# theouterlimitz/Audio-Mastering-Engine

Hardware: AMD Instinct MI355X
Metric: mastered Msamples/sec (48 kHz stereo f32) at 1/2/4/8 GPUs; % HBM roofline (higher is better)
Workload: dtype f64

## Files before the change

### audio-mastering-engine_amd/csrc/amx_dyn.hip

```cpp
#include "amx_dev.hpp"

namespace amx {

typedef double d2v __attribute__((ext_vector_type(2)));
typedef uint32_t u4v __attribute__((ext_vector_type(4)));

#define AMX_TAB 32769

#define AMX_RMS_N 4096
#define AMX_RMS_MAXLOOK 1024

__device__ __forceinline__ int rms_slot(int k) { return k + (k >> 4); }

__device__ __forceinline__ uint32_t rms_floor(uint64_t S, uint32_t cnt, double rc) {
    const double sd = fma((double)(uint32_t)(S >> 32), 4294967296.0, (double)(uint32_t)S);
    const double cd = (double)cnt;
    const uint32_t k = (uint32_t)__builtin_amdgcn_sqrtf((float)(sd * rc));
    const uint32_t k1 = k + 1;
    const bool up = (double)__umul24(k1, k1) * cd <= sd;
    const bool down = (double)__umul24(k, k) * cd > sd;
    const uint32_t r = k + (uint32_t)up - (uint32_t)(down & !up);
    return cnt ? (r > 32768u ? 32768u : r) : 0u;
}

// ... 267 lines not shown
__device__ __forceinline__ void env0_tile(const ChainDev &cd, double *sm, double (&G)[16],
                                          u2v (&Islot)[4], const u2v (&Inext)[4],
                                          const uint16_t *const (&irow)[4], const double *mt, int q,
                                          int ntile, int nwarm, int64_t start, int64_t end,
                                          double *ckr, double &att, double &s_spec, bool &any) {
    const int lane = threadIdx.x & 63;
#pragma unroll
    for (int i = 0; i < 4; i++) {
        double *d = sm + ((lane >> 2) + 16 * i) * AMX_ENV_MP + 4 * (lane & 3);
        *reinterpret_cast<d2v *>(d) = d2v{G[4 * i], G[4 * i + 1]};
        *reinterpret_cast<d2v *>(d + 2) = d2v{G[4 * i + 2], G[4 * i + 3]};
    }
    __builtin_amdgcn_wave_barrier();
    {
        const int qn = (q + AMX_ENV_PF < ntile ? q + AMX_ENV_PF : q) * AMX_ENV_TF;
#pragma unroll
        for (int i = 0; i < 4; i++) Islot[i] = *reinterpret_cast<const u2v *>(irow[i] + qn);
        env_gather(mt, Inext, G);
    }
    const int64_t f0 = start + (int64_t)q * AMX_ENV_TF;
    const bool in = f0 >= 0 && f0 < end;
    double mv[AMX_ENV_TF];
#pragma unroll
    for (int i = 0; i < 8; i++) {
        const d2v v = *reinterpret_cast<const d2v *>(sm + lane * AMX_ENV_MP + 2 * i);
        mv[2 * i] = v.x;
        mv[2 * i + 1] = v.y;
    }
    __builtin_amdgcn_wave_barrier();
    if (q == nwarm) s_spec = att;
    if (in) {
        if (q >= nwarm) {
            ckr[f0 / AMX_ENV_TF] = att;
            uint32_t h = 0, l = 0;
#pragma unroll
            for (int f = 0; f < AMX_ENV_TF; f++) {
                const unsigned long long x = (unsigned long long)__double_as_longlong(mv[f]);
                h |= (uint32_t)(x >> 32);
                l |= (uint32_t)x;
            }
            any |= ((h & 0x7fffffffu) | l) != 0u;
        }
        double iv[AMX_ENV_TF], dv[AMX_ENV_TF];
#pragma unroll
        for (int f = 0; f < AMX_ENV_TF; f++) {
            iv[f] = env_div<RCP>(mv[f], cd.env_A, cd.env_rA);
            dv[f] = env_div<RCP>(mv[f], cd.env_R, cd.env_rR);
        }
#pragma unroll
        for (int f = 0; f < AMX_ENV_TF; f++) att = env_step3(att, mv[f], iv[f], dv[f]);
    }
}

#define AMX_ENV_WG 4
#define AMX_ENV_LDS_PIN (48 * 1024)
template <bool RCP>
__global__ void __launch_bounds__(64 * AMX_ENV_WG) k_env0(const ChainDev *__restrict__ cdp,
                                             const ChunkDev *__restrict__ chunks,
                                             const SegDev *__restrict__ es, int n_es,
                                             const uint16_t *__restrict__ mi,
                                             const double *__restrict__ tabs,
                                             double *__restrict__ ck,
                                             double *__restrict__ sv, double *__restrict__ ev,
                                             int *__restrict__ act, int64_t nloc, int warm,
                                             int *__restrict__ flags) {
    __shared__ __attribute__((aligned(16))) double sm_all[AMX_ENV_WG][64 * AMX_ENV_MP];
    const ChainDev &cd = *cdp;
    const int lane = threadIdx.x & 63, wv = __builtin_amdgcn_readfirstlane(threadIdx.x >> 6);
    double *sm = sm_all[wv];
    if (blockIdx.x == 0 && blockIdx.y == 0 && threadIdx.x < AMX_ENV_MAX_ROUNDS) flags[threadIdx.x] = 0;
    if (blockIdx.x == 0 && blockIdx.y == 0 && threadIdx.x < 64) {
        for (int k = lane; k < AMX_ENV_MAX_ROUNDS * AMX_ENV_NCTR; k += 64) flags[AMX_ENV_MAX_ROUNDS + k] = 0;
        if (lane < 3) flags[AMX_ENV_LIST + lane] = 0;
    }
    const EnvBands eb = env_bands(flags + AMX_ENV_BACT);
    if ((int)blockIdx.y >= eb.nb) return;
    const int b = env_slot_band(eb, blockIdx.y);
    es += cd.etab[eb.nb].es_off;
    n_es = cd.etab[eb.nb].n_es;
    const int Le = cd.etab[eb.nb].Le, ld = cd.es_ld;
    if ((int)(blockIdx.x * (blockDim.x >> 6)) * 64 >= n_es) return;
    const int j = (blockIdx.x * (blockDim.x >> 6) + wv) * 64 + lane;
    const bool valid = j < n_es;
    const SegDev sg = es[valid ? j : n_es - 1];
    const ChunkDev ch = chunks[sg.chunk];
    const int64_t rowoff = b * nloc + ch.loc_off;
    const int64_t start = sg.pos - warm;
    const int64_t end = valid ? sg.pos + sg.len : sg.pos;
    double *ckr = ck + rowoff / AMX_ENV_TF;
    const double *mt = tabs + (int64_t)b * 3 * AMX_TAB;
    const int ntile = (warm + Le) / AMX_ENV_TF, nwarm = warm / AMX_ENV_TF;
    const uint16_t *irow[4];
#pragma unroll
    for (int i = 0; i < 4; i++) {
        const int r = 16 * i + (lane >> 2);
        irow[i] = mi + __shfl(rowoff + start, r) + 4 * (lane & 3);
    }
    u2v I[AMX_ENV_PF][4];
#pragma unroll
    for (int u = 0; u < AMX_ENV_PF; u++)
#pragma unroll
        for (int i = 0; i < 4; i++) I[u][i] = *reinterpret_cast<const u2v *>(irow[i] + u * AMX_ENV_TF);
    double G[2][16];
    env_gather(mt, I[0], G[0]);
    env_gather(mt, I[1], G[1]);
    double att = 0.0, s_spec = 0.0;
    if (cd.env_guess && start >= 0) att = mt[mi[rowoff + start]];
    bool any = false;
    for (int q0 = 0; q0 < ntile; q0 += AMX_ENV_PF) {
#pragma unroll
        for (int u = 0; u < AMX_ENV_PF; u++)
            env0_tile<RCP>(cd, sm, G[u & 1], I[u], I[(u + 2) % AMX_ENV_PF], irow, mt,
                           q0 + u, ntile, nwarm, start, end, ckr, att, s_spec, any);
    }
    if (valid) {
        sv[(int64_t)b * ld + j] = s_spec;
        ev[(int64_t)b * ld + j] = att;
        act[(int64_t)b * ld + j] = any ? 1 : 0;
    }
}

template <bool RCP>
__device__ __forceinline__ double env_fix_segment(const ChainDev &cd, const uint16_t *mrow,
                                                  const double *mt, double *ckr, int64_t pos, int len,
                                                  bool active, double ns, double old_end) {
    if (!active) {
        const int64_t k0 = pos / AMX_ENV_TF_, k1 = (pos + len + AMX_ENV_TF_ - 1) / AMX_ENV_TF_;
        for (int64_t k = k0 + (threadIdx.x & 63); k < k1; k += 64) ckr[k] = ns;
        return ns;
    }
    return env_rerun_wave<RCP>(cd, mrow, mt, ckr, pos, pos + len, ns, old_end);
}

template <bool RCP>
__global__ void __launch_bounds__(64) k_envneed(const ChainDev *__restrict__ cdp,
                                                const SegDev *__restrict__ es, int n_es,
                                                const double *__restrict__ sv,
                                                const double *__restrict__ ev,
                                                const int *__restrict__ act, int *flags,
                                                int *__restrict__ prev, int *__restrict__ list) {
    const ChainDev &cd = *cdp;
    const int b = blockIdx.y, lane = threadIdx.x;
    const EnvBands eb = env_bands(flags + AMX_ENV_BACT);
    if (!eb.act(b)) return;
    es += cd.etab[eb.nb].es_off;
    n_es = cd.etab[eb.nb].n_es;
    const int w0 = blockIdx.x * 64;
    if (w0 >= n_es) return;
    const int j = w0 + lane;
    const bool valid = j < n_es;
    const int64_t bo = (int64_t)b * cd.es_ld;
    const SegDev sg = es[valid ? j : n_es - 1];
    const bool a = valid && act[bo + j] != 0;
    const unsigned long long am = __ballot(a);
    const unsigned long long below = lane ? am & (~0ull >> (64 - lane)) : 0ull;
    int p = below ? w0 + 63 - __clzll((long long)below) : -1;
    if (p < sg.first) p = -1;
    const bool lb = valid && p < 0 && sg.first < w0;
    if (__ballot(lb)) {
        const int first0 = __shfl(sg.first, 0);
        int last = -1;
        for (int base = w0 - 64; base + 63 >= first0; base -= 64) {
            const int jj = base + lane;
            const unsigned long long mk = __ballot(jj >= first0 && act[bo + jj] != 0);
            if (mk) { last = base + 63 - __clzll((long long)mk); break; }
        }
        if (lb) p = last;
    }
    bool need = false;
    if (valid) {
        prev[bo + j] = p;
        need = !((p >= 0 ? ev[bo + p] : 0.0) == sv[bo + j]);
    }
    const unsigned long long nm = __ballot(need);
    if (nm) {
        int base = 0;
        if (lane == 0) base = atomicAdd(flags + AMX_ENV_LIST, __popcll(nm));
        base = __shfl(base, 0);
        const unsigned long long lt = lane ? ~0ull >> (64 - lane) : 0ull;
        if (need) list[base + __popcll(nm & lt)] = (int)(bo + j);
    }
}

template <bool RCP>
__global__ void __launch_bounds__(64) k_envwide(const ChainDev *__restrict__ cdp,
                                                const ChunkDev *__restrict__ chunks,
                                                const SegDev *__restrict__ es,
                                                const uint16_t *__restrict__ mm,
                                                const double *__restrict__ tabs,
                                                double *__restrict__ ck, double *sv, double *ev,
                                                const int *__restrict__ act, int *flags,
                                                const int *__restrict__ prev,
                                                const int *__restrict__ list, int64_t nloc) {
    const int count = __builtin_amdgcn_readfirstlane(flags[AMX_ENV_LIST]);
    if (blockIdx.x == 0 && threadIdx.x == 0) flags[AMX_ENV_MAX_ROUNDS + 3] = count;
    if ((int)blockIdx.x >= count) return;
    const ChainDev &cd = *cdp;
    const int lane = threadIdx.x;
    const EnvBands eb = env_bands(flags + AMX_ENV_BACT);
    const SegDev *et = es + cd.etab[eb.nb].es_off;
    const int ld = cd.es_ld;
    for (int i = blockIdx.x; i < count; i += gridDim.x) {
        const int k = __builtin_amdgcn_readfirstlane(list[i]);
        const int b = k / ld, j = k - b * ld;
        const int64_t bo = (int64_t)b * ld;
        const SegDev sg = et[j];
        const int p = prev[bo + j];
        const double ns = p >= 0 ? ev[bo + p] : 0.0;
        const int64_t ro = b * nloc + chunks[sg.chunk].loc_off;
        const double r = env_fix_segment<RCP>(cd, mm + ro, tabs + (int64_t)b * 3 * AMX_TAB, ck + ro / AMX_ENV_TF_,
                                              sg.pos, sg.len, act[bo + j] != 0, ns, ev[bo + j]);
        __builtin_amdgcn_wave_barrier();
        if (lane == 0) {
            sv[bo + j] = ns;
            ev[bo + j] = r;
        }
    }
}

#ifndef AMX_ENV_CHAIN_WAVES
#define AMX_ENV_CHAIN_WAVES 2048
#endif
template <bool RCP>
__global__ void __launch_bounds__(64) k_envheads(const ChainDev *__restrict__ cdp,
                                                 const SegDev *__restrict__ es, int n_es,
                                                 const double *__restrict__ sv,
                                                 const double *__restrict__ ev,
                                                 int *flags, int *__restrict__ list,
                                                 int *__restrict__ hmark) {
    const ChainDev &cd = *cdp;
    const int b = blockIdx.y, lane = threadIdx.x;
    const EnvBands eb = env_bands(flags + AMX_ENV_BACT);
    if (!eb.act(b)) return;
    es += cd.etab[eb.nb].es_off;
    n_es = cd.etab[eb.nb].n_es;
    if ((int)blockIdx.x * 64 >= n_es) return;
    const int j = blockIdx.x * 64 + lane;
    const int64_t bo = (int64_t)b * cd.es_ld;
    bool head = false;
    if (j < n_es) {
        const int first = es[j].first;
        const bool need = !(sv[bo + j] == (j == first ? 0.0 : ev[bo + j - 1]));
        bool needp = false;
        if (j > first) needp = !(sv[bo + j - 1] == (j - 1 == first ? 0.0 : ev[bo + j - 2]));
        head = need && !needp;
        hmark[bo + j] = head ? 1 : 0;
    }
    const unsigned long long hm = __ballot(head);
    if (hm) {
        int base = 0;
        if (lane == 0) base = atomicAdd(flags + AMX_ENV_LIST + 1, __popcll(hm));
        base = __shfl(base, 0);
        const unsigned long long below = lane ? hm & (~0ull >> (64 - lane)) : 0ull;
        if (head) list[base + __popcll(below)] = (int)(bo + j);
    }
}

template <bool RCP>
__global__ void __launch_bounds__(64) k_envchain(const ChainDev *__restrict__ cdp,
                                                 const ChunkDev *__restrict__ chunks,
                                                 const SegDev *__restrict__ es,
                                                 const uint16_t *__restrict__ mm,
                                                 const double *__restrict__ tabs,
                                                 double *__restrict__ ck, double *sv, double *ev,
                                                 const int *__restrict__ act, int *flags,
                                                 const int *__restrict__ list,
                                                 const int *__restrict__ hmark, int64_t nloc) {
    const int count = __builtin_amdgcn_readfirstlane(flags[AMX_ENV_LIST + 1]);
    if ((int)blockIdx.x >= count) return;
    const ChainDev &cd = *cdp;
    const int lane = threadIdx.x;
    const EnvBands eb = env_bands(flags + AMX_ENV_BACT);
    const SegDev *et = es + cd.etab[eb.nb].es_off;
    const int ld = cd.es_ld;
    int *ctr = flags + AMX_ENV_MAX_ROUNDS;
    int runs = 0, longest = 0, chains = 0;
    bool stale = false;
    const int n_es = cd.etab[eb.nb].n_es;
    for (int i = blockIdx.x; i < count; i += gridDim.x) {
        const int k = __builtin_amdgcn_readfirstlane(list[i]);
        const int b = k / ld, j = k - b * ld;
        const int64_t bo = (int64_t)b * ld;
        const double *mt = tabs + (int64_t)b * 3 * AMX_TAB;
        SegDev sg = et[j];
        const int64_t ro = b * nloc + chunks[sg.chunk].loc_off;
        double *ckr = ck + ro / AMX_ENV_TF_;
        double state = j == sg.first ? 0.0 : ev[bo + j - 1];
        int cur = j, walked = 0;
        bool done = false;
        while (!done) {
            const bool a = act[bo + cur] != 0;
            double old_end = ev[bo + cur];
            const double r = env_fix_segment<RCP>(cd, mm + ro, mt, ckr, sg.pos, sg.len, a, state, old_end);
            walked++;
            __builtin_amdgcn_wave_barrier();
            if (lane == 0) {
                sv[bo + cur] = state;
                ev[bo + cur] = r;
            }
            if (sg.last) break;
            int nx = cur + 1;
            while (true) {
                const int kk = nx + lane;
                const bool inch = kk < n_es && et[kk < n_es ? kk : n_es - 1].first == sg.first;
                bool hk = false, ak = false, st = true;
                double svk = 0.0, evk = 0.0;
                if (inch) {
                    hk = hmark[bo + kk] != 0;
                    ak = act[bo + kk] != 0;
                    svk = sv[bo + kk];
                    evk = ev[bo + kk];
                    st = hk || ak || svk == r;
                }
                const unsigned long long mk = __ballot(st);
                const int f = mk ? __ffsll((long long)mk) - 1 : 64;
                if (f > 0) {
                    const SegDev s0 = et[nx], s1 = et[nx + f - 1];
                    const int64_t k0 = s0.pos / AMX_ENV_TF_, k1 = (s1.pos + s1.len + AMX_ENV_TF_ - 1) / AMX_ENV_TF_;
                    for (int64_t q = k0 + lane; q < k1; q += 64) ckr[q] = r;
                    if (lane < f) {
                        sv[bo + kk] = r;
                        ev[bo + kk] = r;
                    }
                    old_end = __shfl(evk, f - 1);
                    walked += f;
                }
                if (f == 64) {
                    nx += 64;
                    continue;
                }
                const bool ins = __shfl((int)inch, f) != 0, hs = __shfl((int)hk, f) != 0;
                const double ss = __shfl(svk, f);
                if (!ins) { done = true; break; }
                if (hs) {
                    stale = stale || !(r == old_end);
                    done = true;
                    break;
                }
                if (ss == r) { done = true; break; }
                state = r;
                cur = nx + f;
                sg = et[cur];
                break;
            }
        }
        runs += walked;
        longest = walked > longest ? walked : longest;
        chains++;
    }
    if (lane == 0) {
        if (stale) flags[AMX_ENV_LIST + 2] = 1;
        atomicAdd(ctr + 0, runs);
        atomicMax(ctr + 1, longest);
        atomicAdd(ctr + 2, chains);
    }
}

template <bool RCP>
__global__ void __launch_bounds__(64) k_envseq(const ChainDev *__restrict__ cdp,
                                               const ChunkDev *__restrict__ chunks,
                                               const SegDev *__restrict__ es, int n_es,
                                               const int *__restrict__ eseg0,
                                               const int *__restrict__ neseg,
                                               const uint16_t *__restrict__ mm,
                                               const double *__restrict__ tabs,
                                               double *__restrict__ ck,
                                               double *__restrict__ sv, double *__restrict__ ev,
                                               const int *__restrict__ act, int64_t nloc,
                                               const int *__restrict__ flags, int fl) {
    if (fl >= 0 && __builtin_amdgcn_readfirstlane(flags[fl]) == 0) return;
    const ChainDev &cd = *cdp;
    const int c = blockIdx.x, b = blockIdx.y, lane = threadIdx.x;
    const EnvBands eb = env_bands(flags + AMX_ENV_BACT);
    if (!eb.act(b)) return;
    const int tb = eb.nb;
    es += cd.etab[tb].es_off;
    const int s0 = eseg0[cd.etab[tb].ch_off + c], s1 = s0 + neseg[cd.etab[tb].ch_off + c];
    const ChunkDev ch = chunks[c];
    const int64_t ld = cd.es_ld;
    double *S = sv + (int64_t)b * ld, *E = ev + (int64_t)b * ld;
    const int *A = act + (int64_t)b * ld;
    const int64_t ro = b * nloc + ch.loc_off;
    int cur = s0;
    while (cur < s1) {
        int found = s1;
        for (int base = cur; base < s1; base += 64) {
            const int j = base + lane;
            bool bad = false;
            if (j < s1) bad = !((j == s0 ? 0.0 : E[j - 1]) == S[j]);
            const unsigned long long mk = __ballot(bad);
            if (mk) { found = base + __ffsll((long long)mk) - 1; break; }
        }
        if (found >= s1) break;
        const SegDev sg = es[found];
        const double ns = found == s0 ? 0.0 : E[found - 1];
        const double r = env_fix_segment<RCP>(cd, mm + ro, tabs + (int64_t)b * 3 * AMX_TAB,
                                              ck + ro / AMX_ENV_TF_, sg.pos, sg.len, A[found] != 0,
                                              ns, E[found]);
        __syncthreads();
        if (lane == 0) {
            E[found] = r;
            S[found] = ns;
        }
        __threadfence_block();
        __syncthreads();
        cur = found + 1;
    }
}

#define AMX_GO_XP 20
#define AMX_GO_WAVES (AMX_BLOCK / 64)
template <bool RCP>
__global__ void __launch_bounds__(AMX_BLOCK) k_gain_overlay(const ChainDev *__restrict__ cdp,
                                                            const ChunkDev *__restrict__ chunks,
                                                            const uint16_t *__restrict__ mm,
                                                            const double *__restrict__ tabs,
                                                            const double *__restrict__ ck,
                                                            const uint32_t *__restrict__ bands,
                                                            uint32_t *__restrict__ out,
                                                            int64_t nloc,
                                                            const int64_t *__restrict__ n1tab,
                                                            const int *__restrict__ act,
// ... 257 lines not shown
    if (d.look > AMX_RMS_MAXLOOK || C < 1 || C > 8) return hipErrorInvalidValue;
    hipError_t e = launch_zero(bact, 3 * sizeof(int), d.st);
    if (e != hipSuccess) return e;
    const uint32_t *x = reinterpret_cast<const uint32_t *>(bands);
#define MCR(LPV)                                                                                   \
    {                                                                                              \
        constexpr int F = AMX_RMS_N - LPV;                                                         \
        dim3 g((unsigned)((d.max_chunk_n + F - 1) / F), (unsigned)d.n_chunks, 3);                  \
        if (!empty(g))                                                                             \
            hipLaunchKernelGGL(k_mc_rms<LPV>, g, dim3(AMX_BLOCK), 0, d.st, d.cd, d.chunks, schunks, x, \
                               snloc, C, m, d.nloc, bact);                                         \
    }
    if (d.look <= 256) MCR(256) else if (d.look <= 512) MCR(512) else MCR(1024)
#undef MCR
    return hipGetLastError();
}

hipError_t launch_mc_gain_overlay(const DynLaunch &d, const ChunkDev *schunks, const uint16_t *m,
                                  const double *ck, const int16_t *bands, int64_t snloc, int C,
                                  int64_t max_chunk_out, const int64_t *n1tab, const int *bact, int16_t *out) {
    dim3 g((unsigned)((max_chunk_out + AMX_ENV_TF_ * AMX_BLOCK - 1) / (AMX_ENV_TF_ * AMX_BLOCK)),
           (unsigned)d.n_chunks);
    if (empty(g)) return hipSuccess;
    const uint32_t *x = reinterpret_cast<const uint32_t *>(bands);
    if (d.rcp)
        hipLaunchKernelGGL(k_mc_gain_overlay<true>, g, dim3(AMX_BLOCK), 0, d.st, d.cd, d.chunks, schunks, m,
                           d.tabs, ck, x, snloc, d.nloc, C, n1tab, bact, out);
    else
        hipLaunchKernelGGL(k_mc_gain_overlay<false>, g, dim3(AMX_BLOCK), 0, d.st, d.cd, d.chunks, schunks, m,
                           d.tabs, ck, x, snloc, d.nloc, C, n1tab, bact, out);
    return hipGetLastError();
}

template <int LP>
static void rms_t(const DynLaunch &d, const int16_t *bands, uint16_t *m, int *bact) {
    constexpr int N = LP == 256 ? AMX_RMS_N256 : AMX_RMS_N;
    constexpr int F = N - LP;
    dim3 g((unsigned)((d.max_chunk_n + F - 1) / F), (unsigned)d.n_chunks, 3);
    if (empty(g)) return;
    hipLaunchKernelGGL((k_rms<LP, N>), g, dim3(AMX_BLOCK), 0, d.st, d.cd, d.chunks,
                       reinterpret_cast<const uint32_t *>(bands), m, d.nloc, bact);
}

hipError_t launch_rms(const DynLaunch &d, const int16_t *bands, uint16_t *m, int *bact) {
    if (d.look > AMX_RMS_MAXLOOK) return hipErrorInvalidValue;
    if (d.look <= 256) rms_t<256>(d, bands, m, bact);
    else if (d.look <= 512) rms_t<512>(d, bands, m, bact);
    else rms_t<1024>(d, bands, m, bact);
    return hipGetLastError();
}

template <bool RCP>
static void env_launch_t(const DynLaunch &d, const uint16_t *m, double *ck, double *sv, double *ev,
                         int *act, int *list, int *hmark, int *prev, int *list0, int *flags, int rounds,
                         int part) {
    if (part == 0) {
        const int wg = d.env_wg >= 1 && d.env_wg <= AMX_ENV_WG ? d.env_wg : 1;
        const dim3 g0((unsigned)((d.n_es + 64 * wg - 1) / (64 * wg)), 3);
        hipLaunchKernelGGL((k_env0<RCP>), g0, dim3(64 * wg), d.env_pin ? AMX_ENV_LDS_PIN : 0, d.st, d.cd,
                           d.chunks, d.es, d.n_es, m, d.tabs, ck, sv, ev, act, d.nloc, d.warm, flags);
        return;
    }
    if (rounds <= 0) return;
    const dim3 gs((unsigned)((d.n_es + 63) / 64), 3);
    hipLaunchKernelGGL(k_envneed<RCP>, gs, dim3(64), 0, d.st, d.cd, d.es, d.n_es, sv, ev, act, flags, prev, list0);
    hipLaunchKernelGGL(k_envwide<RCP>, dim3(AMX_ENV_CHAIN_WAVES), dim3(64), 0, d.st, d.cd, d.chunks, d.es, m,
                       d.tabs, ck, sv, ev, act, flags, prev, list0, d.nloc);
    hipLaunchKernelGGL(k_envheads<RCP>, dim3((unsigned)((d.n_es + 63) / 64), 3), dim3(64), 0, d.st, d.cd, d.es,
                       d.n_es, sv, ev, flags, list, hmark);
    hipLaunchKernelGGL(k_envchain<RCP>, dim3(AMX_ENV_CHAIN_WAVES), dim3(64), 0, d.st, d.cd, d.chunks, d.es, m,
                       d.tabs, ck, sv, ev, act, flags, list, hmark, d.nloc);
}

hipError_t launch_env(const DynLaunch &d, const uint16_t *m, double *ck, double *sv, double *ev,
                      int *act, int *list, int *hmark, int *prev, int *list0, int *flags, int rounds,
                      int part) {
    if (d.n_es <= 0) return hipSuccess;
    if (d.warm % (AMX_ENV_TF * AMX_ENV_PF) || d.Le % (AMX_ENV_TF * AMX_ENV_PF))
        return hipErrorInvalidValue;
    if (rounds < 0 || rounds > AMX_ENV_MAX_ROUNDS) return hipErrorInvalidValue;
    if (d.rcp) env_launch_t<true>(d, m, ck, sv, ev, act, list, hmark, prev, list0, flags, rounds, part);
    else env_launch_t<false>(d, m, ck, sv, ev, act, list, hmark, prev, list0, flags, rounds, part);
    return hipGetLastError();
}

hipError_t launch_envseq(const DynLaunch &d, const uint16_t *m, double *ck, double *sv, double *ev,
                         const int *act, const int *flags, int rounds) {
    if (d.n_es <= 0) return hipSuccess;
    const dim3 gr((unsigned)d.n_chunks, 3);
    const int fl = rounds > 0 ? AMX_ENV_LIST + 2 : -1;
    if (d.rcp)
        hipLaunchKernelGGL(k_envseq<true>, gr, dim3(64), 0, d.st, d.cd, d.chunks, d.es, d.n_es,
                           d.eseg0, d.neseg, m, d.tabs, ck, sv, ev, act, d.nloc, flags, fl);
    else
        hipLaunchKernelGGL(k_envseq<false>, gr, dim3(64), 0, d.st, d.cd, d.chunks, d.es, d.n_es,
                           d.eseg0, d.neseg, m, d.tabs, ck, sv, ev, act, d.nloc, flags, fl);
    return hipGetLastError();
}

hipError_t launch_gain_overlay(const DynLaunch &d, const uint16_t *m, const double *ck,
                               const int16_t *bands, int16_t *out, int64_t max_chunk_out,
                               const int64_t *n1tab, const int *act, const int *bact) {
    dim3 g((unsigned)((max_chunk_out + AMX_ENV_TF_ * AMX_BLOCK - 1) / (AMX_ENV_TF_ * AMX_BLOCK)),
           (unsigned)d.n_chunks);
    if (empty(g)) return hipSuccess;
    const uint32_t *x = reinterpret_cast<const uint32_t *>(bands);
    uint32_t *o = reinterpret_cast<uint32_t *>(out);
    if (d.rcp)
        hipLaunchKernelGGL(k_gain_overlay<true>, g, dim3(AMX_BLOCK), 0, d.st, d.cd, d.chunks, m, d.tabs, ck,
                           x, o, d.nloc, n1tab, act, d.eseg0, d.neseg, act ? 1 : 0, bact);
    else
        hipLaunchKernelGGL(k_gain_overlay<false>, g, dim3(AMX_BLOCK), 0, d.st, d.cd, d.chunks, m, d.tabs, ck,
                           x, o, d.nloc, n1tab, act, d.eseg0, d.neseg, act ? 1 : 0, bact);
    return hipGetLastError();
}

}
```

### audio-mastering-engine_amd/csrc/amx_internal.hpp

```cpp
#pragma once
#include <hip/hip_runtime.h>
#include <stdint.h>

#include "amx_tables.hpp"

#define AMX_BLOCK 256
#define AMX_HIST_BINS 1000
#define AMX_SCAN_PW 6
#define AMX_CTL_FAST 1
#define AMX_STATS 16
#ifndef AMX_PCM_U8
#define AMX_PCM_U8 0
#define AMX_PCM_S16 1
#define AMX_PCM_S24 2
#define AMX_PCM_S32 3
#define AMX_PCM_F32 4
#define AMX_PCM_F64 5
#define AMX_PCM_S8 6
#define AMX_PCM_S16BE 7
#define AMX_PCM_S24BE 8
#define AMX_PCM_S32BE 9
#define AMX_PCM_F32BE 10
#define AMX_PCM_F64BE 11
#endif
// ... 16 lines not shown
    const ScanBlk *blks;
    const double *M;
    const double *Mbk;
};
hipError_t launch_front1(const Launch &l, int D, int win, bool analog, const float *in,
                         const float *lut, int16_t *a16, const double *G, double *e, bool sc = false);
hipError_t launch_scan(const ScanPlan &p, const double *e, double *s, const double *carry,
                       double *eb, hipStream_t st, bool up = true, const double *tailP = nullptr,
                       double *tail = nullptr);
hipError_t launch_front2(const Launch &l, int mask, const int16_t *a16, const double *s_eq,
                         int16_t *dst, int to_out, const double *Gx, double *e_x,
                         const double *Gkw, double *e_kw, uint32_t *pk, bool sc = false,
                         const float *slut = nullptr);
hipError_t launch_xover2(const Launch &l, const int16_t *p16, const double *s_x,
                         int16_t *bands, int64_t nloc, int *bact);
struct DynLaunch {
    const ChainDev *cd;
    const ChunkDev *chunks;
    int n_chunks;
    const SegDev *es;
    int n_es;
    const int *eseg0, *neseg;
    int64_t nloc, max_chunk_n;
    int look, warm, Le, rcp;
    const double *tabs;
    hipStream_t st;
    int env_wg, env_pin;
};
hipError_t launch_rms(const DynLaunch &d, const int16_t *bands, uint16_t *m, int *bact);
hipError_t launch_mc_rms(const DynLaunch &d, const ChunkDev *schunks, const int16_t *bands, int64_t snloc,
                         int C, uint16_t *m, int *bact);
hipError_t launch_mc_gain_overlay(const DynLaunch &d, const ChunkDev *schunks, const uint16_t *m,
                                  const double *ck, const int16_t *bands, int64_t snloc, int C,
                                  int64_t max_chunk_out, const int64_t *n1tab, const int *bact, int16_t *out);
hipError_t launch_mc_pack(const void *in, int64_t samples, int in_s16, uint32_t *pairs, hipStream_t st);
hipError_t launch_mc_unpack(const uint32_t *pairs, int64_t samples, int16_t *out, hipStream_t st);
hipError_t launch_mc_split_pairs(const int16_t *y, int64_t frames, int C, int16_t *pairs, hipStream_t st);
hipError_t launch_mc_loudness_combine(const double *hops, int64_t max_hops, const double *peak, int C,
                                      double *hops1, double *peak1, hipStream_t st);
hipError_t launch_mc_peak_pick(const int16_t *y, int64_t frames, int C, const double *gain, int16_t *syn,
                               hipStream_t st);
hipError_t launch_mc_limiter_out(const int16_t *y, int64_t frames, int C, int halo_frames, const double *gains,
                                 const int32_t *ctl, const double *att, double level_in, double level,
                                 double level_out, double limit, int16_t *out, hipStream_t st);
hipError_t launch_zero(void *p, size_t bytes, hipStream_t st);
hipError_t launch_pcm_to_s16(const void *raw, int64_t frames, int channels, int fmt, int16_t *out,
                             hipStream_t st);
void flac_encode_size(int64_t frames, int C, int B, int lpc_order, int64_t *nf, int64_t *max_out,
                      int64_t *ws_bytes);
hipError_t launch_flac_encode(const int16_t *pcm, int64_t frames, int C, int fs, int B, int lpc_order, uint8_t *out,
                              int64_t capacity, uint32_t *frame_bytes, uint32_t *sub_bits, int64_t *total,
                              void *ws, hipStream_t st);
hipError_t launch_env(const DynLaunch &d, const uint16_t *m, double *ck, double *sv, double *ev,
                      int *act, int *list, int *hmark, int *prev, int *list0, int *flags, int rounds,
                      int part);
hipError_t launch_envseq(const DynLaunch &d, const uint16_t *m, double *ck, double *sv, double *ev,
                         const int *act, const int *flags, int rounds);
hipError_t launch_gain_overlay(const DynLaunch &d, const uint16_t *m, const double *ck,
                               const int16_t *bands, int16_t *out, int64_t max_chunk_out,
                               const int64_t *n1tab, const int *act, const int *bact);
hipError_t launch_kw1(const ChainDev *cd, const KwSegDev *ks, int n_kseg, int L,
                      const int16_t *x, const double *G, double *e, uint32_t *pk,
                      const int32_t *gate, hipStream_t st);
hipError_t launch_kw2(const ChainDev *cd, const KwSegDev *ks, int n_kseg, int L, int hop,
                      const int16_t *x, const double *s, double *parts, int64_t *part_hop,
                      int aligned, const int32_t *gate, hipStream_t st);
hipError_t launch_hops(const SpanDev *spans, int n_tracks, const KwSegDev *ks, int L, int hop,
                       const double *parts, const int64_t *part_hop, double *hops,
                       int64_t max_hops, hipStream_t st);
hipError_t launch_hist(const SpanDev *spans, int n_tracks, int hop, const double *hops,
                       int64_t max_hops, const double *bounds, unsigned long long *hist,
                       unsigned long long *st_hist, hipStream_t st);
#define AMX_UP_EDGE 80
#define AMX_UP_BLOCK 64
struct UpArgs {
    const ChainDev *cd;
    const KwSegDev *ks;
    int n_kseg;
    const SpanDev *spans;
    int Lin, Lout;
    int static_l;
    int poly;
    const int32_t *fcnt;
    const float *bankn;
    int hop;
    const int32_t *obase, *oph;
    const float *owt;
    int lin;
    const int32_t *slow;
    int64_t n_slow;
    const float *bank;
    int taps, alloc;
    const uint32_t *x, *edge;
    const double *G;
    const double *qh, *qt;
    double *eterms;
    double *e;
    const double *s;
    double *parts;
    int64_t *part_hop;
    uint32_t *pk;
};
struct LnArgs {
    int64_t n192;
    float *u;
    double *ring;
    int16_t *y;
    double *summary;
    const double *hops;
    const double *peak;
// ... 108 lines not shown
```

### audio-mastering-engine_amd/csrc/amx_plan.cpp

```cpp
#include "../../include/amx.h"
#include "amx_internal.hpp"
#include "amx_plan.hpp"

#include <algorithm>
#include <climits>
#include <cmath>
#include <cstdio>
#include <cstdarg>
#include <cstdlib>
#include <cstring>
#include <memory>
#include <string>
#include <vector>

namespace {

thread_local std::string g_err;

int fail(int code, const char *fmt, ...) {
    char buf[512];
    va_list ap;
    va_start(ap, fmt);
    vsnprintf(buf, sizeof buf, fmt, ap);
    va_end(ap);
// ... 168 lines not shown
    if (p->up_aux) (void)hipStreamDestroy(p->up_aux);
    delete p;
}

int amx_plan_get_info(const amx_plan *p, amx_plan_info *info) {
    if (!p || !info) return fail(AMX_EINVAL, "null argument");
    memset(info, 0, sizeof *info);
    info->workspace_bytes = (int64_t)p->ws_bytes;
    info->out_frames = p->out_frames;
    info->n_tracks = p->n_tracks;
    info->n_chunks = p->n_chunks;
    info->n_segments = p->n_seg;
    info->seg_frames = p->L;
    info->scan_levels_eq = p->lev_eq;
    info->scan_levels_xover = p->lev_x;
    info->scan_levels_kw = p->lev_kw;
    info->eq_dim = p->D;
    info->hop_frames = p->hop;
    info->meas_rate = p->meas_native ? p->cd.fs : AMX_MEAS_RATE;
    info->max_hops = p->max_hops;
    return AMX_OK;
}

int amx_plan_track_span(const amx_plan *p, int32_t track, amx_track_span *span) {
    if (!p || !span || track < 0 || track >= p->n_tracks) return fail(AMX_EINVAL, "bad track");
    const SpanDev &s = p->spans[track];
    span->out_offset = s.out_off;
    span->out_frames = s.out_n;
    span->track_frame0 = s.tframe0;
    span->track_frames_total = s.ttotal;
    return AMX_OK;
}

int amx_run_stage(amx_plan *p, int32_t stage, const float *d_in, int16_t *d_out, void *d_ws,
                  void *stream) {
    if (!p || (p->nloc > 0 && (!d_in || !d_out || !d_ws))) return fail(AMX_EINVAL, "null argument");
    if (stage < 0 || stage >= AMX_STAGE_COUNT) return fail(AMX_EINVAL, "bad stage %d", stage);
    if (p->n_seg == 0) return AMX_OK;
    hipStream_t st = (hipStream_t)stream;
    amx::Launch l{p->d_cd, p->d_chunks, p->d_segs, p->n_chunks, p->n_seg, p->L, st, p->d_lut_half,
                  p->f1_mode, p->max_chunk_n, p->an_blocks, p->an_vec};
    int16_t *a16 = wsp<int16_t>(d_ws, p->o_a16);
    double *e = wsp<double>(d_ws, p->o_e), *s = wsp<double>(d_ws, p->o_s);
    int16_t *p16 = p->mb ? wsp<int16_t>(d_ws, p->o_p16) : nullptr;
    double *ex = p->mb ? wsp<double>(d_ws, p->o_ex) : nullptr;
    double *sx = p->mb ? wsp<double>(d_ws, p->o_sx) : nullptr;
    int16_t *bands = p->mb ? wsp<int16_t>(d_ws, p->o_bands) : nullptr;
    double *ck = p->mb ? wsp<double>(d_ws, p->o_gain) : nullptr;
    uint16_t *mframe = p->mb ? wsp<uint16_t>(d_ws, p->o_m) : nullptr;
    double *esv = p->mb ? wsp<double>(d_ws, p->o_esv) : nullptr;
    double *ee0 = p->mb ? wsp<double>(d_ws, p->o_ee0) : nullptr;
    int *eflags = p->mb ? wsp<int>(d_ws, p->o_eflags) : nullptr;
    int *eact = p->mb ? wsp<int>(d_ws, p->o_eact) : nullptr;
    int *ehead = p->mb ? wsp<int>(d_ws, p->o_ehead) : nullptr;
    int *elist = p->mb ? wsp<int>(d_ws, p->o_elist) : nullptr;
    int *eprev = p->mb ? wsp<int>(d_ws, p->o_eprev) : nullptr;
    int *elist0 = p->mb ? wsp<int>(d_ws, p->o_elist0) : nullptr;
    amx::DynLaunch dl{p->d_cd,    p->d_chunks, p->n_chunks, p->d_esegs, p->n_es,
                      p->d_eseg0, p->d_neseg,  p->nloc,     p->max_chunk_n, p->cd.look,
                      p->warm,    p->Le,       p->cd.env_rcp, p->d_tabs, st,
                      p->env_wg,  p->env_pin};
    switch (stage) {
    case AMX_STAGE_FRONT1:
        if (p->mono16) {
            int16_t *dup = wsp<int16_t>(d_ws, p->o_dup);
            HIPCHK(amx::launch_pcm_to_s16(d_in, p->in_frames, 1, AMX_PCM_S16, dup, st));
            d_in = reinterpret_cast<const float *>(dup);
        }
        HIPCHK(amx::launch_front1(l, p->D, (p->cd.chin == 2 && !p->cd.in_s16) ? 2 : 1,
                                  p->cd.analog_on != 0, d_in, p->sc ? p->d_in_lut : p->d_lut, a16, p->d_G, e,
                                  p->sc != 0));
        break;
    case AMX_STAGE_SCAN_EQ:
        if (p->D > 0)
            HIPCHK(amx::launch_scan(p->scan_eq(), e, s, nullptr, wsp<double>(d_ws, p->o_eb), st));
        break;
    case AMX_STAGE_FRONT2:
        if (p->mb)
            HIPCHK(amx::launch_front2(l, p->mask, a16, s, p16, 0, p->d_Gx, ex, nullptr, nullptr,
                                      nullptr, p->sc != 0, p->d_in_lut));
        else if (p->sc)
            HIPCHK(amx::launch_front2(l, p->mask, a16, s, d_out, 1, nullptr, nullptr, nullptr,
                                      nullptr, nullptr, true, p->d_in_lut));
        else if (p->fuse_kw)
            HIPCHK(amx::launch_front2(l, p->mask, a16, s, d_out, 1, nullptr, nullptr, p->d_Gkw,
                                      wsp<double>(d_ws, p->o_ekw), wsp<uint32_t>(d_ws, p->o_pk)));
        else
            HIPCHK(amx::launch_front2(l, p->mask, a16, s, d_out, 1, nullptr, nullptr, nullptr,
                                      nullptr, nullptr));
        break;
    case AMX_STAGE_SCAN_XO:
        if (p->mb)
            HIPCHK(amx::launch_scan(p->scan_xo(), ex, sx, nullptr, wsp<double>(d_ws, p->o_ebx), st));
        break;
    case AMX_STAGE_XOVER:
        if (p->mb) HIPCHK(amx::launch_xover2(l, p16, sx, bands, p->nloc, eflags + AMX_ENV_BACT));
        break;
    case AMX_STAGE_RMS:
        if (p->mb) HIPCHK(amx::launch_rms(dl, bands, mframe, eflags + AMX_ENV_BACT));
        break;
    case AMX_STAGE_ENV:
        if (p->mb)
            HIPCHK(amx::launch_env(dl, mframe, ck, esv, ee0, eact, elist, ehead, eprev, elist0, eflags, p->rounds, 0));
        break;
    case AMX_STAGE_FIX:
        if (p->mb) {
            HIPCHK(amx::launch_env(dl, mframe, ck, esv, ee0, eact, elist, ehead, eprev, elist0, eflags, p->rounds, 1));
            HIPCHK(amx::launch_envseq(dl, mframe, ck, esv, ee0, eact, eflags, p->rounds));
        }
        break;
    case AMX_STAGE_APPLY:
        if (p->mb)
            HIPCHK(amx::launch_gain_overlay(dl, mframe, ck, bands, d_out, p->max_chunk_out, p->d_n1, eact,
                                            eflags + AMX_ENV_BACT));
        break;
    }
    return AMX_OK;
}

int amx_run_chunks(amx_plan *p, const float *d_in, int16_t *d_out, void *d_ws, void *stream) {
    for (int s = 0; s < AMX_STAGE_COUNT; s++) {
        int rc = amx_run_stage(p, s, d_in, d_out, d_ws, stream);
        if (rc) return rc;
    }
    return AMX_OK;
}

}

namespace {
amx::UpArgs up_args(const amx_plan *p, const int16_t *d_out, const int16_t *d_edge, void *d_ws) {
    amx::UpArgs a{};
    a.cd = p->d_cd;
    a.ks = p->d_ksegs;
    a.n_kseg = p->n_kseg;
    a.spans = p->d_spans;
    a.Lin = p->upLin;
    a.Lout = p->upLout;
    a.static_l = p->up_static;
    a.poly = p->up_poly;
    a.fcnt = p->d_fcnt;
    a.bankn = p->d_bankn;
    a.hop = p->hop;
    a.obase = p->d_obase;
    a.oph = p->d_oph;
    a.owt = p->d_owt;
    a.lin = p->up_lin;
    a.slow = p->d_slow;
    a.n_slow = p->n_slow;
    a.bank = p->d_bank;
    a.taps = p->up_taps;
    a.alloc = p->up_alloc;
    a.x = reinterpret_cast<const uint32_t *>(d_out);
    a.edge = reinterpret_cast<const uint32_t *>(d_edge);
    a.G = p->d_Gkw;
    a.qh = p->d_qh;
    a.qt = p->d_qt;
    a.eterms = wsp<double>(d_ws, p->o_eterms);
    a.e = wsp<double>(d_ws, p->o_ekw);
    a.s = wsp<double>(d_ws, p->o_skw);
// ... 872 lines not shown
```

Before: 32150.

## Fold envelope need/head detection into env0 and fixup kernels via per-wave summaries

Removes the separate k_envneed and k_envheads passes. k_env0 now writes per-segment marks, resolved start states and per-wave summaries (entry count, last active lane, end state). k_envwide and k_envchain rebuild their work lists from these summaries with wave-wide prefix scans instead of atomic-appended lists. The aim is to cut two kernel launches and their global passes over sv/ev/act. In exchange the design is more complex, relies on reusing old workspace slots for the new arrays and on 7-bit count packing, and every envwide block rescans the full summary array.

```diff
diff --git a/audio-mastering-engine_amd/csrc/amx_dyn.hip b/audio-mastering-engine_amd/csrc/amx_dyn.hip
--- a/audio-mastering-engine_amd/csrc/amx_dyn.hip
+++ b/audio-mastering-engine_amd/csrc/amx_dyn.hip
@@ -343,6 +343,61 @@
     }
 }
 
+#define AMX_EM_CHANGED 1
+#define AMX_EM_RERUN 2
+#define AMX_EM_DONE 4
+#define AMX_EM_KIND(m) (((m) >> 4) & 3)
+#define AMX_EM_BOUNDARY 1
+#define AMX_EM_RESOLVED 2
+
+struct EnvHand {
+    int *mark, *ns_lo, *ns_hi, *wsum;
+    double *wend;
+};
+__host__ __device__ __forceinline__ int env_wend_off(int ld) { return (3 * ((ld + 63) / 64) + 1) & ~1; }
+
+__device__ __forceinline__ int wave_incl_scan(int v) {
+    const int lane = threadIdx.x & 63;
+#pragma unroll
+    for (int o = 1; o < 64; o <<= 1) {
+        const int up = __shfl_up(v, o);
+        if (lane >= o) v += up;
+    }
+    return v;
+}
+
+__device__ __forceinline__ void env0_hand_off(const EnvHand &h, int64_t bo, int tw, bool later_wave,
+                                              int j0, bool valid, int first, double s_spec,
+                                              double end, bool any) {
+    const int lane = threadIdx.x & 63;
+    const bool a = valid && any;
+    const unsigned long long am = __ballot(a);
+    const unsigned long long lt = lane ? ~0ull >> (64 - lane) : 0ull;
+    const unsigned long long below = am & lt;
+    int pl = below ? 63 - __clzll((long long)below) : -1;
+    if (j0 + pl < first) pl = -1;
+    const double pe = __shfl(end, pl >= 0 ? pl : 0);
+    const bool unresolved = valid && pl < 0 && first < j0;
+    const double ns = pl >= 0 ? pe : 0.0;
+    const bool need = valid && !unresolved && !(ns == s_spec);
+    const int kind = unresolved ? AMX_EM_BOUNDARY : need ? AMX_EM_RESOLVED : 0;
+    if (valid) {
+        h.mark[bo + j0 + lane] = kind << 4;
+        if (need) {
+            const long long x = __double_as_longlong(ns);
+            h.ns_lo[bo + j0 + lane] = (int)x;
+            h.ns_hi[bo + j0 + lane] = (int)(x >> 32);
+        }
+    }
+    const int ll = am ? 63 - __clzll((long long)am) : -1;
+    const double le = __shfl(end, ll >= 0 ? ll : 0);
+    const int nent = __popcll(__ballot(kind != 0)), nres = __popcll(__ballot(need));
+    if (lane == 0) {
+        h.wsum[tw] = nent | (ll + 1) << 8 | nres << 16;
+        if (later_wave) h.wend[tw] = le;
+    }
+}
+
 #define AMX_ENV_WG 4
 #define AMX_ENV_LDS_PIN (48 * 1024)
 template <bool RCP>
@@ -354,7 +409,7 @@
                                              double *__restrict__ ck,
                                              double *__restrict__ sv, double *__restrict__ ev,
                                              int *__restrict__ act, int64_t nloc, int warm,
-                                             int *__restrict__ flags) {
+                                             int *__restrict__ flags, EnvHand hand) {
     __shared__ __attribute__((aligned(16))) double sm_all[AMX_ENV_WG][64 * AMX_ENV_MP];
     const ChainDev &cd = *cdp;
     const int lane = threadIdx.x & 63, wv = __builtin_amdgcn_readfirstlane(threadIdx.x >> 6);
@@ -409,6 +464,10 @@
         ev[(int64_t)b * ld + j] = att;
         act[(int64_t)b * ld + j] = any ? 1 : 0;
     }
+    const int j0 = j - lane;
+    if (j0 < n_es)
+        env0_hand_off(hand, (int64_t)b * ld, (int)blockIdx.y * ((n_es + 63) / 64) + j0 / 64, j0 + 64 < n_es,
+                      j0, valid, sg.first, s_spec, att, any);
 }
 
 template <bool RCP>
@@ -423,54 +482,72 @@
     return env_rerun_wave<RCP>(cd, mrow, mt, ckr, pos, pos + len, ns, old_end);
 }
 
-template <bool RCP>
-__global__ void __launch_bounds__(64) k_envneed(const ChainDev *__restrict__ cdp,
-                                                const SegDev *__restrict__ es, int n_es,
-                                                const double *__restrict__ sv,
-                                                const double *__restrict__ ev,
-                                                const int *__restrict__ act, int *flags,
-                                                int *__restrict__ prev, int *__restrict__ list) {
-    const ChainDev &cd = *cdp;
-    const int b = blockIdx.y, lane = threadIdx.x;
-    const EnvBands eb = env_bands(flags + AMX_ENV_BACT);
-    if (!eb.act(b)) return;
-    es += cd.etab[eb.nb].es_off;
-    n_es = cd.etab[eb.nb].n_es;
-    const int w0 = blockIdx.x * 64;
-    if (w0 >= n_es) return;
-    const int j = w0 + lane;
-    const bool valid = j < n_es;
-    const int64_t bo = (int64_t)b * cd.es_ld;
-    const SegDev sg = es[valid ? j : n_es - 1];
-    const bool a = valid && act[bo + j] != 0;
-    const unsigned long long am = __ballot(a);
-    const unsigned long long below = lane ? am & (~0ull >> (64 - lane)) : 0ull;
-    int p = below ? w0 + 63 - __clzll((long long)below) : -1;
-    if (p < sg.first) p = -1;
-    const bool lb = valid && p < 0 && sg.first < w0;
-    if (__ballot(lb)) {
-        const int first0 = __shfl(sg.first, 0);
-        int last = -1;
-        for (int base = w0 - 64; base + 63 >= first0; base -= 64) {
-            const int jj = base + lane;
-            const unsigned long long mk = __ballot(jj >= first0 && act[bo + jj] != 0);
-            if (mk) { last = base + 63 - __clzll((long long)mk); break; }
-        }
-        if (lb) p = last;
-    }
-    bool need = false;
-    if (valid) {
-        prev[bo + j] = p;
-        need = !((p >= 0 ? ev[bo + p] : 0.0) == sv[bo + j]);
-    }
-    const unsigned long long nm = __ballot(need);
-    if (nm) {
-        int base = 0;
-        if (lane == 0) base = atomicAdd(flags + AMX_ENV_LIST, __popcll(nm));
-        base = __shfl(base, 0);
-        const unsigned long long lt = lane ? ~0ull >> (64 - lane) : 0ull;
-        if (need) list[base + __popcll(nm & lt)] = (int)(bo + j);
-    }
+
+struct EnvMap {
+    int nt, R, sum, incl, total;
+};
+__device__ __forceinline__ EnvMap env_map(const int *__restrict__ wsum, int nt, int &nres) {
+    const int lane = threadIdx.x & 63;
+    EnvMap m;
+    m.nt = nt;
+    m.R = (nt + 63) / 64;
+    int s = 0, q = 0;
+#pragma unroll 4
+    for (int r = 0; r < m.R; r++) {
+        const int t = lane * m.R + r;
+        const int w = t < nt ? wsum[t] : 0;
+        s += w & 127;
+        q += (w >> 16) & 127;
+    }
+    m.sum = s;
+    m.incl = wave_incl_scan(s);
+    m.total = __shfl(m.incl, 63);
+    nres = q;
+    return m;
+}
+__device__ __forceinline__ void env_map_find(const EnvMap &m, const int *__restrict__ wsum, int i,
+                                             int &t, int &k) {
+    const int lane = threadIdx.x & 63;
+    const int l = __ffsll((long long)__ballot(i < m.incl)) - 1;
+    int rem = i - (__shfl(m.incl, l) - __shfl(m.sum, l));
+    const int t0 = l * m.R;
+    t = -1;
+    k = 0;
+    for (int r0 = 0; r0 < m.R; r0 += 64) {
+        const int tt = t0 + r0 + lane;
+        const int c = (r0 + lane < m.R && tt < m.nt) ? wsum[tt] & 127 : 0;
+        const int incl = wave_incl_scan(c);
+        const int tot = __shfl(incl, 63);
+        if (rem < tot) {
+            const int l2 = __ffsll((long long)__ballot(rem < incl)) - 1;
+            t = t0 + r0 + l2;
+            k = rem - (__shfl(incl, l2) - __shfl(c, l2));
+            return;
+        }
+        rem -= tot;
+    }
+}
+struct EnvEntry {
+    int slot, w, b, j, mark;
+    int64_t bo;
+};
+__device__ __forceinline__ EnvEntry env_entry(const EnvBands &eb, const int *mark, int ld, int n_es,
+                                              int nw, int t, int k) {
+    const int lane = threadIdx.x & 63;
+    EnvEntry e;
+    e.slot = t / nw;
+    e.w = t - e.slot * nw;
+    e.b = env_slot_band(eb, e.slot);
+    e.bo = (int64_t)e.b * ld;
+    const int jj = e.w * 64 + lane;
+    const int mk = (t >= 0 && jj < n_es) ? mark[e.bo + jj] : 0;
+    const unsigned long long em = __ballot(AMX_EM_KIND(mk) != 0);
+    const unsigned long long lt = lane ? ~0ull >> (64 - lane) : 0ull;
+    const unsigned long long sel = __ballot(((em >> lane) & 1) && __popcll(em & lt) == k);
+    const int L = sel ? __ffsll((long long)sel) - 1 : 0;
+    e.j = sel ? e.w * 64 + L : -1;
+    e.mark = __shfl(mk, L);
+    return e;
 }
 
 template <bool RCP>
@@ -480,71 +557,75 @@
                                                 const uint16_t *__restrict__ mm,
                                                 const double *__restrict__ tabs,
                                                 double *__restrict__ ck, double *sv, double *ev,
-                                                const int *__restrict__ act, int *flags,
-                                                const int *__restrict__ prev,
-                                                const int *__restrict__ list, int64_t nloc) {
-    const int count = __builtin_amdgcn_readfirstlane(flags[AMX_ENV_LIST]);
-    if (blockIdx.x == 0 && threadIdx.x == 0) flags[AMX_ENV_MAX_ROUNDS + 3] = count;
-    if ((int)blockIdx.x >= count) return;
+                                                const int *__restrict__ act, int *flags, EnvHand h,
+                                                int64_t nloc) {
     const ChainDev &cd = *cdp;
     const int lane = threadIdx.x;
     const EnvBands eb = env_bands(flags + AMX_ENV_BACT);
+    if (eb.nb == 0) return;
     const SegDev *et = es + cd.etab[eb.nb].es_off;
-    const int ld = cd.es_ld;
-    for (int i = blockIdx.x; i < count; i += gridDim.x) {
-        const int k = __builtin_amdgcn_readfirstlane(list[i]);
-        const int b = k / ld, j = k - b * ld;
-        const int64_t bo = (int64_t)b * ld;
-        const SegDev sg = et[j];
-        const int p = prev[bo + j];
-        const double ns = p >= 0 ? ev[bo + p] : 0.0;
-        const int64_t ro = b * nloc + chunks[sg.chunk].loc_off;
-        const double r = env_fix_segment<RCP>(cd, mm + ro, tabs + (int64_t)b * 3 * AMX_TAB, ck + ro / AMX_ENV_TF_,
-                                              sg.pos, sg.len, act[bo + j] != 0, ns, ev[bo + j]);
+    const int n_es = cd.etab[eb.nb].n_es, ld = cd.es_ld, nw = (n_es + 63) / 64;
+    int q;
+    const EnvMap map = env_map(h.wsum, eb.nb * nw, q);
+    int nre = 0;
+    if (blockIdx.x == 0) nre = __shfl(wave_incl_scan(q), 63);
+    for (int i = blockIdx.x; i < map.total; i += gridDim.x) {
+        int t, k;
+        env_map_find(map, h.wsum, i, t, k);
+        const EnvEntry e = env_entry(eb, h.mark, ld, n_es, nw, t, k);
+        if (e.j < 0) continue;
+        const int kind = AMX_EM_KIND(e.mark);
+        if (e.mark & AMX_EM_DONE) {
+            nre += kind == AMX_EM_BOUNDARY && (e.mark & AMX_EM_RERUN);
+            continue;
+        }
+        const int64_t bj = e.bo + e.j;
+        const SegDev sg = et[e.j];
+        double ns = 0.0;
+        if (kind == AMX_EM_RESOLVED) {
+            ns = __longlong_as_double((long long)h.ns_hi[bj] << 32 | (unsigned)h.ns_lo[bj]);
+        } else {
+            const int wf = sg.first >> 6;
+            for (int base = e.w - 64; base + 63 >= wf; base -= 64) {
+                const int ww = base + lane;
+                const int word = ww >= 0 ? h.wsum[e.slot * nw + ww] : 0;
+                const unsigned long long mk = __ballot(((word >> 8) & 127) != 0);
+                if (mk) {
+                    const int hl = 63 - __clzll((long long)mk);
+                    const int wp = base + hl;
+                    const int p = wp * 64 + ((__shfl(word, hl) >> 8) & 127) - 1;
+                    if (p >= sg.first) ns = h.wend[e.slot * nw + wp];
+                    break;
+                }
+            }
+            if (ns == sv[bj]) {
+                if (lane == 0) h.mark[bj] = e.mark | AMX_EM_DONE;
+                continue;
+            }
+            nre++;
+        }
+        const double old_end = ev[bj];
+        const int64_t ro = e.b * nloc + chunks[sg.chunk].loc_off;
+        const double r = env_fix_segment<RCP>(cd, mm + ro, tabs + (int64_t)e.b * 3 * AMX_TAB, ck + ro / AMX_ENV_TF_,
+                                              sg.pos, sg.len, act[bj] != 0, ns, old_end);
         __builtin_amdgcn_wave_barrier();
         if (lane == 0) {
-            sv[bo + j] = ns;
-            ev[bo + j] = r;
-        }
-    }
+            sv[bj] = ns;
+            ev[bj] = r;
+            h.mark[bj] = e.mark | AMX_EM_DONE | AMX_EM_RERUN | (r == old_end ? 0 : AMX_EM_CHANGED);
+        }
+    }
+    if (lane == 0 && nre) atomicAdd(flags + AMX_ENV_LIST, nre);
 }
 
 #ifndef AMX_ENV_CHAIN_WAVES
 #define AMX_ENV_CHAIN_WAVES 2048
 #endif
-template <bool RCP>
-__global__ void __launch_bounds__(64) k_envheads(const ChainDev *__restrict__ cdp,
-                                                 const SegDev *__restrict__ es, int n_es,
-                                                 const double *__restrict__ sv,
-                                                 const double *__restrict__ ev,
-                                                 int *flags, int *__restrict__ list,
-                                                 int *__restrict__ hmark) {
-    const ChainDev &cd = *cdp;
-    const int b = blockIdx.y, lane = threadIdx.x;
-    const EnvBands eb = env_bands(flags + AMX_ENV_BACT);
-    if (!eb.act(b)) return;
-    es += cd.etab[eb.nb].es_off;
-    n_es = cd.etab[eb.nb].n_es;
-    if ((int)blockIdx.x * 64 >= n_es) return;
-    const int j = blockIdx.x * 64 + lane;
-    const int64_t bo = (int64_t)b * cd.es_ld;
-    bool head = false;
-    if (j < n_es) {
-        const int first = es[j].first;
-        const bool need = !(sv[bo + j] == (j == first ? 0.0 : ev[bo + j - 1]));
-        bool needp = false;
-        if (j > first) needp = !(sv[bo + j - 1] == (j - 1 == first ? 0.0 : ev[bo + j - 2]));
-        head = need && !needp;
-        hmark[bo + j] = head ? 1 : 0;
-    }
-    const unsigned long long hm = __ballot(head);
-    if (hm) {
-        int base = 0;
-        if (lane == 0) base = atomicAdd(flags + AMX_ENV_LIST + 1, __popcll(hm));
-        base = __shfl(base, 0);
-        const unsigned long long below = lane ? hm & (~0ull >> (64 - lane)) : 0ull;
-        if (head) list[base + __popcll(below)] = (int)(bo + j);
-    }
+__device__ __forceinline__ bool env_chain_start(const int *__restrict__ act, const int *mark, int64_t bo,
+                                                int k, int first) {
+    const bool c1 = act[bo + k - 1] != 0 && (mark[bo + k - 1] & AMX_EM_CHANGED);
+    const bool c2 = k - 2 >= first && act[bo + k - 2] != 0 && (mark[bo + k - 2] & AMX_EM_CHANGED);
+    return c1 && !c2;
 }
 
 template <bool RCP>
@@ -554,29 +635,35 @@
                                                  const uint16_t *__restrict__ mm,
                                                  const double *__restrict__ tabs,
                                                  double *__restrict__ ck, double *sv, double *ev,
-                                                 const int *__restrict__ act, int *flags,
-                                                 const int *__restrict__ list,
-                                                 const int *__restrict__ hmark, int64_t nloc) {
-    const int count = __builtin_amdgcn_readfirstlane(flags[AMX_ENV_LIST + 1]);
-    if ((int)blockIdx.x >= count) return;
+                                                 const int *__restrict__ act, int *flags, EnvHand h,
+                                                 int64_t nloc) {
     const ChainDev &cd = *cdp;
     const int lane = threadIdx.x;
     const EnvBands eb = env_bands(flags + AMX_ENV_BACT);
+    if (eb.nb == 0) return;
     const SegDev *et = es + cd.etab[eb.nb].es_off;
-    const int ld = cd.es_ld;
+    const int n_es = cd.etab[eb.nb].n_es, ld = cd.es_ld, nw = (n_es + 63) / 64;
     int *ctr = flags + AMX_ENV_MAX_ROUNDS;
+    if (blockIdx.x == 0 && lane == 0) ctr[3] = flags[AMX_ENV_LIST];
     int runs = 0, longest = 0, chains = 0;
     bool stale = false;
-    const int n_es = cd.etab[eb.nb].n_es;
-    for (int i = blockIdx.x; i < count; i += gridDim.x) {
-        const int k = __builtin_amdgcn_readfirstlane(list[i]);
-        const int b = k / ld, j = k - b * ld;
-        const int64_t bo = (int64_t)b * ld;
+    for (int t = blockIdx.x; t < eb.nb * nw; t += gridDim.x) {
+      const int slot = t / nw, w = t - slot * nw, b = env_slot_band(eb, slot);
+      const int64_t bo = (int64_t)b * ld;
+      const int jj = w * 64 + lane;
+      unsigned long long cm = __ballot(jj < n_es && (h.mark[bo + jj] & AMX_EM_CHANGED) && act[bo + jj] != 0);
+      while (cm) {
+        const int p = w * 64 + __ffsll((long long)cm) - 1;
+        cm &= cm - 1;
+        SegDev sg = et[p];
+        if (sg.last || !env_chain_start(act, h.mark, bo, p + 1, sg.first)) continue;
+        const int j = p + 1;
+        double state = ev[bo + p];
+        if (sv[bo + j] == state) continue;
         const double *mt = tabs + (int64_t)b * 3 * AMX_TAB;
-        SegDev sg = et[j];
         const int64_t ro = b * nloc + chunks[sg.chunk].loc_off;
         double *ckr = ck + ro / AMX_ENV_TF_;
-        double state = j == sg.first ? 0.0 : ev[bo + j - 1];
+        sg = et[j];
         int cur = j, walked = 0;
         bool done = false;
         while (!done) {
@@ -597,7 +684,7 @@
                 bool hk = false, ak = false, st = true;
                 double svk = 0.0, evk = 0.0;
                 if (inch) {
-                    hk = hmark[bo + kk] != 0;
+                    hk = env_chain_start(act, h.mark, bo, kk, sg.first);
                     ak = act[bo + kk] != 0;
                     svk = sv[bo + kk];
                     evk = ev[bo + kk];
@@ -638,8 +725,9 @@
         runs += walked;
         longest = walked > longest ? walked : longest;
         chains++;
-    }
-    if (lane == 0) {
+      }
+    }
+    if (lane == 0 && chains) {
         if (stale) flags[AMX_ENV_LIST + 2] = 1;
         atomicAdd(ctr + 0, runs);
         atomicMax(ctr + 1, longest);
@@ -658,7 +746,8 @@
                                                double *__restrict__ ck,
                                                double *__restrict__ sv, double *__restrict__ ev,
                                                const int *__restrict__ act, int64_t nloc,
-                                               const int *__restrict__ flags, int fl) {
+                                               int *flags, int fl) {
+    if (blockIdx.x == 0 && blockIdx.y == 0 && threadIdx.x == 0) flags[AMX_ENV_LIST] = 0;
     if (fl >= 0 && __builtin_amdgcn_readfirstlane(flags[fl]) == 0) return;
     const ChainDev &cd = *cdp;
     const int c = blockIdx.x, b = blockIdx.y, lane = threadIdx.x;
@@ -1022,40 +1111,36 @@
 
 template <bool RCP>
 static void env_launch_t(const DynLaunch &d, const uint16_t *m, double *ck, double *sv, double *ev,
-                         int *act, int *list, int *hmark, int *prev, int *list0, int *flags, int rounds,
-                         int part) {
+                         int *act, const EnvHand &h, int *flags, int rounds, int part) {
     if (part == 0) {
         const int wg = d.env_wg >= 1 && d.env_wg <= AMX_ENV_WG ? d.env_wg : 1;
         const dim3 g0((unsigned)((d.n_es + 64 * wg - 1) / (64 * wg)), 3);
         hipLaunchKernelGGL((k_env0<RCP>), g0, dim3(64 * wg), d.env_pin ? AMX_ENV_LDS_PIN : 0, d.st, d.cd,
-                           d.chunks, d.es, d.n_es, m, d.tabs, ck, sv, ev, act, d.nloc, d.warm, flags);
+                           d.chunks, d.es, d.n_es, m, d.tabs, ck, sv, ev, act, d.nloc, d.warm, flags, h);
         return;
     }
     if (rounds <= 0) return;
-    const dim3 gs((unsigned)((d.n_es + 63) / 64), 3);
-    hipLaunchKernelGGL(k_envneed<RCP>, gs, dim3(64), 0, d.st, d.cd, d.es, d.n_es, sv, ev, act, flags, prev, list0);
     hipLaunchKernelGGL(k_envwide<RCP>, dim3(AMX_ENV_CHAIN_WAVES), dim3(64), 0, d.st, d.cd, d.chunks, d.es, m,
-                       d.tabs, ck, sv, ev, act, flags, prev, list0, d.nloc);
-    hipLaunchKernelGGL(k_envheads<RCP>, dim3((unsigned)((d.n_es + 63) / 64), 3), dim3(64), 0, d.st, d.cd, d.es,
-                       d.n_es, sv, ev, flags, list, hmark);
+                       d.tabs, ck, sv, ev, act, flags, h, d.nloc);
     hipLaunchKernelGGL(k_envchain<RCP>, dim3(AMX_ENV_CHAIN_WAVES), dim3(64), 0, d.st, d.cd, d.chunks, d.es, m,
-                       d.tabs, ck, sv, ev, act, flags, list, hmark, d.nloc);
+                       d.tabs, ck, sv, ev, act, flags, h, d.nloc);
 }
 
 hipError_t launch_env(const DynLaunch &d, const uint16_t *m, double *ck, double *sv, double *ev,
-                      int *act, int *list, int *hmark, int *prev, int *list0, int *flags, int rounds,
+                      int *act, int *mark, int *ns_lo, int *ns_hi, int *wsum, int *flags, int rounds,
                       int part) {
     if (d.n_es <= 0) return hipSuccess;
     if (d.warm % (AMX_ENV_TF * AMX_ENV_PF) || d.Le % (AMX_ENV_TF * AMX_ENV_PF))
         return hipErrorInvalidValue;
     if (rounds < 0 || rounds > AMX_ENV_MAX_ROUNDS) return hipErrorInvalidValue;
-    if (d.rcp) env_launch_t<true>(d, m, ck, sv, ev, act, list, hmark, prev, list0, flags, rounds, part);
-    else env_launch_t<false>(d, m, ck, sv, ev, act, list, hmark, prev, list0, flags, rounds, part);
+    const EnvHand h{mark, ns_lo, ns_hi, wsum, reinterpret_cast<double *>(wsum + env_wend_off(d.n_es))};
+    if (d.rcp) env_launch_t<true>(d, m, ck, sv, ev, act, h, flags, rounds, part);
+    else env_launch_t<false>(d, m, ck, sv, ev, act, h, flags, rounds, part);
     return hipGetLastError();
 }
 
 hipError_t launch_envseq(const DynLaunch &d, const uint16_t *m, double *ck, double *sv, double *ev,
-                         const int *act, const int *flags, int rounds) {
+                         const int *act, int *flags, int rounds) {
     if (d.n_es <= 0) return hipSuccess;
     const dim3 gr((unsigned)d.n_chunks, 3);
     const int fl = rounds > 0 ? AMX_ENV_LIST + 2 : -1;
diff --git a/audio-mastering-engine_amd/csrc/amx_internal.hpp b/audio-mastering-engine_amd/csrc/amx_internal.hpp
--- a/audio-mastering-engine_amd/csrc/amx_internal.hpp
+++ b/audio-mastering-engine_amd/csrc/amx_internal.hpp
@@ -92,10 +92,10 @@
                               int64_t capacity, uint32_t *frame_bytes, uint32_t *sub_bits, int64_t *total,
                               void *ws, hipStream_t st);
 hipError_t launch_env(const DynLaunch &d, const uint16_t *m, double *ck, double *sv, double *ev,
-                      int *act, int *list, int *hmark, int *prev, int *list0, int *flags, int rounds,
+                      int *act, int *mark, int *ns_lo, int *ns_hi, int *wsum, int *flags, int rounds,
                       int part);
 hipError_t launch_envseq(const DynLaunch &d, const uint16_t *m, double *ck, double *sv, double *ev,
-                         const int *act, const int *flags, int rounds);
+                         const int *act, int *flags, int rounds);
 hipError_t launch_gain_overlay(const DynLaunch &d, const uint16_t *m, const double *ck,
                                const int16_t *bands, int16_t *out, int64_t max_chunk_out,
                                const int64_t *n1tab, const int *act, const int *bact);
diff --git a/audio-mastering-engine_amd/csrc/amx_plan.cpp b/audio-mastering-engine_amd/csrc/amx_plan.cpp
--- a/audio-mastering-engine_amd/csrc/amx_plan.cpp
+++ b/audio-mastering-engine_amd/csrc/amx_plan.cpp
@@ -244,10 +244,10 @@
     double *ee0 = p->mb ? wsp<double>(d_ws, p->o_ee0) : nullptr;
     int *eflags = p->mb ? wsp<int>(d_ws, p->o_eflags) : nullptr;
     int *eact = p->mb ? wsp<int>(d_ws, p->o_eact) : nullptr;
-    int *ehead = p->mb ? wsp<int>(d_ws, p->o_ehead) : nullptr;
-    int *elist = p->mb ? wsp<int>(d_ws, p->o_elist) : nullptr;
-    int *eprev = p->mb ? wsp<int>(d_ws, p->o_eprev) : nullptr;
-    int *elist0 = p->mb ? wsp<int>(d_ws, p->o_elist0) : nullptr;
+    int *emark = p->mb ? wsp<int>(d_ws, p->o_ehead) : nullptr;
+    int *ens_lo = p->mb ? wsp<int>(d_ws, p->o_elist) : nullptr;
+    int *ens_hi = p->mb ? wsp<int>(d_ws, p->o_eprev) : nullptr;
+    int *ewsum = p->mb ? wsp<int>(d_ws, p->o_elist0) : nullptr;
     amx::DynLaunch dl{p->d_cd,    p->d_chunks, p->n_chunks, p->d_esegs, p->n_es,
                       p->d_eseg0, p->d_neseg,  p->nloc,     p->max_chunk_n, p->cd.look,
                       p->warm,    p->Le,       p->cd.env_rcp, p->d_tabs, st,
@@ -293,11 +293,11 @@
         break;
     case AMX_STAGE_ENV:
         if (p->mb)
-            HIPCHK(amx::launch_env(dl, mframe, ck, esv, ee0, eact, elist, ehead, eprev, elist0, eflags, p->rounds, 0));
+            HIPCHK(amx::launch_env(dl, mframe, ck, esv, ee0, eact, emark, ens_lo, ens_hi, ewsum, eflags, p->rounds, 0));
         break;
     case AMX_STAGE_FIX:
         if (p->mb) {
-            HIPCHK(amx::launch_env(dl, mframe, ck, esv, ee0, eact, elist, ehead, eprev, elist0, eflags, p->rounds, 1));
+            HIPCHK(amx::launch_env(dl, mframe, ck, esv, ee0, eact, emark, ens_lo, ens_hi, ewsum, eflags, p->rounds, 1));
             HIPCHK(amx::launch_envseq(dl, mframe, ck, esv, ee0, eact, eflags, p->rounds));
         }
         break;
```

After: 32120. Within noise of the previous version (-0.1%).
